# rvp-group/mad-icp

Hardware: NVIDIA H100
Metric: scans/sec (130k-pt scan vs 16-keyframe model) (higher is better)
Workload: dtype f64

## Files before the change

mad_icp_b200/csrc/capi.cu:

```cuda
#include <cooperative_groups.h>
#include <cuda_runtime.h>

#include <algorithm>
#include <cmath>
#include <cstdio>
#include <cstdlib>
#include <cstring>
#include <new>
#include <stdexcept>
#include <string>
#include <vector>

#include "../../include/madicp_b200_debug.h"
#include "ctx.hpp"
#include "device_kernels.cuh"

namespace madicp {

static thread_local std::string g_error;
void set_error(const std::string& msg) { g_error = msg; }

}

using namespace madicp;
// ... 59 lines not shown
  DevPtr<double> ww;
  const size_t total = cap * size_t(c->max_keyframes);
  CK(cudaMalloc(recs.put(), total * sizeof(madtree_rec_t)));
  CK(cudaMalloc(child0.put(), total * sizeof(int)));
  CK(cudaMalloc(rec_of.put(), total * sizeof(int)));
  CK(cudaMalloc(quad.put(), 2 * total * sizeof(QuadRec)));
  CK(cudaMalloc(ww.put(), total * sizeof(double)));
  for (int s = 0; s < c->max_keyframes; ++s)
    if (c->slots[s].n_nodes > 0)
      CK(cudaMemcpyAsync(recs + size_t(s) * cap, c->d_pool_recs + size_t(s) * c->pool_cap,
                         size_t(c->slots[s].n_nodes) * sizeof(madtree_rec_t), cudaMemcpyDeviceToDevice, c->stream));
  CK(cudaStreamSynchronize(c->stream));
  c->d_pool_ww = std::move(ww);
  c->d_pool_recs = std::move(recs);
  c->d_pool_child0 = std::move(child0);
  c->d_pool_rec_of = std::move(rec_of);
  c->d_quad = std::move(quad);
  c->quad_cap = 2 * cap;
  c->pool_cap = cap;
  for (int s = 0; s < c->max_keyframes; ++s)
    if (c->slots[s].n_nodes > 0) {
      int rc = build_slot(c, s, nullptr, nullptr);
      if (rc) return rc;
    }
  return MADICP_OK;
}

static int stage_pose(madicp_ctx* c, const double X[12], const double** X_dev) {
  const int r = int(c->xform_seq % madicp_ctx::kXformRing);
  if (c->xform_seq >= madicp_ctx::kXformRing) CK(cudaEventSynchronize(c->xform_done[r]));
  memcpy(c->h_xform + size_t(r) * 12, X, 12 * sizeof(double));
  CK(cudaMemcpyAsync(c->d_xform + size_t(r) * 12, c->h_xform + size_t(r) * 12, 12 * sizeof(double), cudaMemcpyHostToDevice,
                     c->stream));
  CK(cudaEventRecord(c->xform_done[r], c->stream));
  *X_dev = c->d_xform + size_t(r) * 12;
  c->xform_seq++;
  return MADICP_OK;
}

static int slot_rank(const madicp_ctx* c, int slot) {
  int k = 0;
  for (int s = 0; s < slot; ++s) k += (c->slots[s].n_nodes > 0);
  return k;
}

static int ensure_items(madicp_ctx* c, size_t items) {
  if (items <= c->cap_items) return MADICP_OK;
  CK(cudaStreamSynchronize(c->stream));
  c->cap_items = 0;
  CK(cudaMalloc(c->d_hit.put(), items * sizeof(int)));
  CK(cudaMalloc(c->d_ord.put(), items * sizeof(int)));
  c->cap_items = items;
  return MADICP_OK;
}

struct GnShape {
  int threads, ctas;
  const void* fn;
  size_t smem;
};
template <int THREADS, int CTAS>
static GnShape gn_shape() {
  return GnShape{THREADS, CTAS, reinterpret_cast<const void*>(k_gn_loop<THREADS, CTAS>), gn_dynamic_smem<THREADS>()};
}
static const GnShape* gn_shapes(int* n) {
  static const GnShape table[] = {
      gn_shape<1024, 1>(), gn_shape<896, 1>(), gn_shape<768, 1>(), gn_shape<704, 1>(), gn_shape<640, 1>(),
      gn_shape<512, 1>(),  gn_shape<512, 2>(),
      gn_shape<256, 2>(),  gn_shape<256, 3>(), gn_shape<256, 4>(),
  };
  *n = int(sizeof(table) / sizeof(table[0]));
  return table;
}
static int configure_gn(madicp_ctx* c, int threads, int ctas) {
  int n = 0;
  const GnShape* t = gn_shapes(&n);
  for (int i = 0; i < n; ++i)
    if (t[i].threads == threads && t[i].ctas == ctas) {
      CK(cudaFuncSetAttribute(t[i].fn, cudaFuncAttributeMaxDynamicSharedMemorySize, int(t[i].smem + kGnMapMaxBytes)));
      CK(cudaFuncSetAttribute(t[i].fn, cudaFuncAttributePreferredSharedMemoryCarveout,
                              int((t[i].smem * size_t(ctas) + 2048) * 100 / (228 * 1024)) + 1));
      int per_sm = 0;
      CK(cudaOccupancyMaxActiveBlocksPerMultiprocessor(&per_sm, t[i].fn, threads, t[i].smem));
      if (per_sm < ctas) {
        set_error("persistent kernel shape does not fit on an SM");
        return MADICP_ERR_CUDA;
      }
      c->gn_threads = threads;
      c->gn_grid = ctas * c->sm_count;
      c->gn_kernel = t[i].fn;
      c->gn_smem = t[i].smem;
      return MADICP_OK;
    }
  set_error("unsupported persistent-kernel shape (threads per CTA, CTAs per SM)");
  return MADICP_ERR_INVALID;
}

static int pick_shape(madicp_ctx* c, int64_t items) {
  if (!c->gn_auto) return MADICP_OK;
  const double per_sm = double((items + 31) / 32) / double(c->sm_count);
  int best = 1024;
  double best_cost = 1e300;
  for (int i = 0; i < madicp_ctx::kNumAutoShapes; ++i) {
    const int threads = madicp_ctx::kAutoShapes[i];
    const double passes = ceil(per_sm / double(threads / 32));
    const double cost = passes * c->pass_cost[i];
    if (cost < best_cost) {
      best_cost = cost;
      best = threads;
    }
  }
  if (best == c->gn_threads && c->gn_grid == c->sm_count) return MADICP_OK;
  return configure_gn(c, best, 1);
}

static int grid_for(const madicp_ctx* c, int64_t items) {
  int64_t g = (items + kStepBlock - 1) / kStepBlock;
  const int64_t cap = int64_t(c->sm_count) * 8;
  if (g > cap) g = cap;
  if (g < 1) g = 1;
  return int(g);
}

madicp_ctx::~madicp_ctx() {
  cudaSetDevice(device);
  if (stream) cudaStreamSynchronize(stream);
  for (int r = 0; r < world; ++r)
    if (world > 1 && r != rank && peer_comm[r]) cudaIpcCloseMemHandle(peer_comm[r]);
  madicp_gpu_build_release(this);
  for (madtree_gpu* t : tree_cache) delete t;
  for (CloudBuf* b : cloud_cache) delete b;
}

extern "C" {

const char* madicp_last_error(void) { return g_error.c_str(); }
int madicp_abi_version(void) { return 3; }

int madicp_create(madicp_ctx_t** out, int device, int max_keyframes) {
  if (!out || max_keyframes < 1 || max_keyframes > kMaxSlots) {
    set_error("madicp_create: bad arguments (1 <= max_keyframes <= 64)");
    return MADICP_ERR_INVALID;
  }
  MADICP_TRY
  int n_dev = 0;
  cudaError_t e = cudaGetDeviceCount(&n_dev);
  if (e != cudaSuccess || n_dev <= 0 || device < 0 || device >= n_dev) {
    set_error(std::string("madicp_create: no usable CUDA device (") +
              (e != cudaSuccess ? cudaGetErrorString(e) : "device index out of range") +
              "); this library has no CPU fallback");
    return MADICP_ERR_CUDA;
  }
  CK(cudaSetDevice(device));
  cudaDeviceProp prop;
  CK(cudaGetDeviceProperties(&prop, device));
  if (prop.major != 9 || prop.minor != 0) {
    set_error("madicp_create: device is not sm_90 (H100); kernels are built for sm_90a only");
    return MADICP_ERR_CUDA;
  }
  std::unique_ptr<madicp_ctx> c(new madicp_ctx);
  c->device = device;
  c->max_keyframes = max_keyframes;
  c->sm_count = prop.multiProcessorCount;
  c->slots.resize(max_keyframes);
  {
    int lo_pri = 0, hi_pri = 0;
    CK(cudaDeviceGetStreamPriorityRange(&lo_pri, &hi_pri));
    CK(cudaStreamCreateWithPriority(c->own_stream.put(), cudaStreamNonBlocking, hi_pri));
  }
  c->stream = c->own_stream;
  CK(cudaMalloc(c->d_state.put(), sizeof(GnState)));
  CK(cudaMemset(c->d_state, 0, sizeof(GnState)));
  CK(cudaMalloc(c->d_X.put(), sizeof(double) * 64));
  CK(cudaMalloc(c->d_comm.put(), sizeof(CommBlock)));
// ... 749 lines not shown
  }
  memcpy(c->h_pinned, X, 12 * sizeof(double));
  CK(cudaMemcpyAsync(c->d_X, c->h_pinned, 12 * sizeof(double), cudaMemcpyHostToDevice, c->stream));
  rc = launch_search(c, mv, c->d_X, false);
  if (rc) return rc;
  CK(cudaMemsetAsync(c->d_state, 0, 16, c->stream));
  CK(cudaMemsetAsync(c->d_step_matched, 0, size_t(c->L), c->stream));
  const int64_t items = int64_t(mv.K) * c->L;
  const int grid = grid_for(c, items);
  k_linearize<<<grid, kStepBlock, 0, c->stream>>>(mv, c->d_mov4, c->L, c->d_X, c->P, c->d_hit, c->d_step_matched,
                                                 c->d_partial, c->d_state);
  c->launches++;
  CK(cudaGetLastError());
  CK(cudaMemcpyAsync(c->h_state, c->d_state, offsetof(GnState, X_trace), cudaMemcpyDeviceToHost, c->stream));
  if (matched) CK(cudaMemcpyAsync(c->h_matched, c->d_step_matched, size_t(c->L), cudaMemcpyDeviceToHost, c->stream));
  CK(cudaStreamSynchronize(c->stream));
  memcpy(H, c->h_state->H, sizeof(double) * 36);
  memcpy(b, c->h_state->b, sizeof(double) * 6);
  if (matched) memcpy(matched, c->h_matched, size_t(c->L));
  return MADICP_OK;
}

int madicp_solve_update(madicp_ctx_t* c, const double H[36], const double b[6], double X[12]) {
  if (!c || !H || !b || !X) return MADICP_ERR_INVALID;
  CK(cudaSetDevice(c->device));
  memcpy(c->h_pinned, X, 12 * sizeof(double));
  memcpy(c->h_pinned + 12, H, 36 * sizeof(double));
  memcpy(c->h_pinned + 48, b, 6 * sizeof(double));
  CK(cudaMemcpyAsync(c->d_X, c->h_pinned, 54 * sizeof(double), cudaMemcpyHostToDevice, c->stream));
  k_solve<<<1, 32, 0, c->stream>>>(c->d_X + 12, c->d_X + 48, c->d_X);
  c->launches++;
  CK(cudaGetLastError());
  CK(cudaMemcpyAsync(c->h_pinned, c->d_X, 12 * sizeof(double), cudaMemcpyDeviceToHost, c->stream));
  CK(cudaStreamSynchronize(c->stream));
  memcpy(X, c->h_pinned, 12 * sizeof(double));
  return MADICP_OK;
}

int madicp_debug_inv_det6(madicp_ctx_t* c, const double H[36], double* weight) {
  if (!c || !H || !weight) return MADICP_ERR_INVALID;
  CK(cudaSetDevice(c->device));
  memcpy(c->h_pinned + 12, H, 36 * sizeof(double));
  CK(cudaMemcpyAsync(c->d_X + 12, c->h_pinned + 12, 36 * sizeof(double), cudaMemcpyHostToDevice, c->stream));
  k_inv_det6<<<1, 32, 0, c->stream>>>(c->d_X + 12, c->d_X + 48);
  c->launches++;
  CK(cudaGetLastError());
  CK(cudaMemcpyAsync(c->h_pinned + 48, c->d_X + 48, sizeof(double), cudaMemcpyDeviceToHost, c->stream));
  CK(cudaStreamSynchronize(c->stream));
  *weight = c->h_pinned[48];
  return MADICP_OK;
}

static int register_enqueue(madicp_ctx* c, int iters, const double X0[12], int clear_from) {
  int rc = check_ready(c, "madicp_register");
  if (rc) return rc;
  if (!X0 || iters < 1 || iters > MADICP_MAX_ITERS) {
    set_error("madicp_register: bad arguments (1 <= iters <= 64 per launch)");
    return MADICP_ERR_INVALID;
  }
  CK(cudaSetDevice(c->device));
  rc = prepare_moving(c);
  if (rc) return rc;
  rc = pick_shape(c, int64_t(madicp_num_keyframes(c)) * c->L);
  if (rc) return rc;
  GnArgs A;
  A.model = make_view(c);
  A.P = c->P;
  A.peers.rank = c->rank;
  A.peers.world = c->world;
  A.peers.epoch_base = c->epoch;
  const int mb = int(c->call_seq & 1u);
  for (int r = 0; r < kMaxPeers; ++r) {
    A.peers.box[r] = (r < c->world) ? &c->peer_comm[r]->box : nullptr;
    A.peer_matched[r] = (r < c->world) ? c->peer_comm[r]->matched[mb] : nullptr;
  }
  A.moving = c->d_mov4;
  A.L = c->L;
  A.iters = iters;
  A.clear_from = clear_from;
  A.matched = c->d_comm->matched[mb];
  size_t map_bytes = 0;
  {
    const size_t per_cta = gn_map_bytes(unsigned(madicp_num_keyframes(c)), unsigned(c->L), unsigned(c->gn_grid));
    auto bucket = [](size_t bytes) {
      const size_t kb[] = {8, 16, 32, 64, 100, 132, 164, 196, 228};
      for (size_t b : kb)
        if (bytes + 1024 <= b * 1024) return b;
      return size_t(1 << 20);
    };
    const size_t ctas = size_t(c->gn_grid / c->sm_count);
    if (per_cta && bucket((c->gn_smem + per_cta) * ctas) == bucket(c->gn_smem * ctas)) map_bytes = per_cta;
  }
  A.map_in_smem = map_bytes ? 1 : 0;
  {
    const size_t stride =
        ((size_t(c->max_keyframes) * gn_share_bound(c->cap_moving, unsigned(c->gn_grid))) + 31) & ~size_t(31);
    const size_t need = stride * size_t(c->gn_grid);
    if (need > c->cap_memo) {
      CK(cudaStreamSynchronize(c->stream));
      c->cap_memo = 0;
      const size_t cap = need + need / 4;
      CK(cudaMalloc(c->d_memo_leaf.put(), cap * sizeof(int)));
      CK(cudaMalloc(c->d_memo_margin.put(), cap * sizeof(float)));
      CK(cudaMalloc(c->d_memo_ckpt.put(), cap * sizeof(unsigned)));
      CK(cudaMalloc(c->d_memo_ckpt_up.put(), cap * sizeof(float)));
      c->cap_memo = cap;
    }
    A.memo_leaf = c->d_memo_leaf;
    A.memo_margin = c->d_memo_margin;
    A.memo_ckpt = c->d_memo_ckpt;
    A.memo_ckpt_up = c->d_memo_ckpt_up;
    A.item_stride = int(stride);
    A.memo_mode = c->memo_mode;
    A.walk_buf = mb;
  }
  A.st = c->d_state;
  A.dbg = c->d_dbg;
  A.dbg_cta = c->d_dbg ? c->d_dbg_cta.get() : nullptr;
  c->epoch += uint32_t(iters);
  A.pose_epoch = c->pose_epoch;
  c->pose_epoch += uint32_t(iters);
  memcpy(A.X0, X0, 12 * sizeof(double));
  A.tiles = c->d_tiles;
  A.zero_next = c->d_comm->matched[mb ^ 1];
  A.zero_bytes = int((std::min(kMatchedCap, c->cap_moving) + 15) & ~size_t(15));
  void* args[] = {&A};
  CK(cudaLaunchCooperativeKernel(c->gn_kernel, dim3(c->gn_grid), dim3(c->gn_threads), args, c->gn_smem + map_bytes, c->stream));
  c->launches++;
  c->last_iters = iters;
  c->call_seq++;
  return MADICP_OK;
}

int madicp_register_async(madicp_ctx_t* c, int iters, const double X0[12]) {
  return register_enqueue(c, iters, X0, iters - 1);
}
int madicp_register_partial_async(madicp_ctx_t* c, int iters, const double X0[12]) {
  return register_enqueue(c, iters, X0, 0);
}

int madicp_register_fetch_weight(madicp_ctx_t* c, double X[12], double H[36], double b[6], uint8_t* matched, int* n_matched,
                                 double* weight) {
  if (!c || c->last_iters < 1) {
    set_error("madicp_register_fetch: nothing was enqueued");
    return MADICP_ERR_STATE;
  }
  CK(cudaSetDevice(c->device));
  CK(cudaMemcpyAsync(c->h_state, c->d_state, offsetof(GnState, X_trace), cudaMemcpyDeviceToHost, c->stream));
  if (matched)
    CK(cudaMemcpyAsync(c->h_matched, c->d_comm->matched[(c->call_seq - 1u) & 1u], size_t(c->L), cudaMemcpyDeviceToHost,
                       c->stream));
  CK(cudaStreamSynchronize(c->stream));
  if (c->h_state->error) {
    set_error("madicp_register: a peer GPU never delivered its H/b tile (rank down, or no matching registration enqueued there)");
    CK(cudaMemsetAsync(&c->d_state->error, 0, sizeof(int), c->stream));
    return MADICP_ERR_COMM;
  }
  if (X) memcpy(X, c->h_state->X_out, 12 * sizeof(double));
  if (H) memcpy(H, c->h_state->H, 36 * sizeof(double));
  if (b) memcpy(b, c->h_state->b, 6 * sizeof(double));
  if (matched) memcpy(matched, c->h_matched, size_t(c->L));
  if (n_matched) *n_matched = c->h_state->n_matched;
  if (weight) *weight = c->h_state->weight;
  return MADICP_OK;
}
int madicp_register_fetch(madicp_ctx_t* c, double X[12], double H[36], double b[6], uint8_t* matched, int* n_matched) {
  return madicp_register_fetch_weight(c, X, H, b, matched, n_matched, nullptr);
}

int madicp_register(madicp_ctx_t* c, int iters, double X[12], double H[36], double b[6], uint8_t* matched,
                    int* n_matched) {
  if (!c || !X || iters < 0) {
    set_error("madicp_register: bad arguments");
    return MADICP_ERR_INVALID;
// ... 291 lines not shown
```

mad_icp_b200/csrc/ctx.hpp:

```cpp
#pragma once
#include <cuda_runtime.h>

#include <atomic>
#include <memory>
#include <mutex>
#include <new>
#include <stdexcept>
#include <string>
#include <vector>

#include "cuda_owned.hpp"
#include "kernels.cuh"

namespace madicp {
void set_error(const std::string& msg);

constexpr int kMaxLevels = 4096;
struct Slot {
  int n_nodes = 0, n_leaves = 0, n_levels = 0;
};
constexpr size_t kMatchedCap = size_t(1) << 20;

struct CommBlock {
  Mailbox box;
// ... 24 lines not shown
  std::shared_ptr<madicp::CloudBuf> cloud;
  int64_t cloud_off = 0;
};

struct madicp_ctx {
  ~madicp_ctx();
  int device = 0;
  int max_keyframes = 0;
  madicp::Stream own_stream;
  cudaStream_t stream = nullptr;
  int sm_count = 0;
  std::vector<madicp::Slot> slots;
  size_t pool_cap = 0;
  madicp::DevPtr<madtree_rec_t> d_pool_recs;
  madicp::DevPtr<int> d_pool_child0;
  madicp::DevPtr<int> d_pool_rec_of;
  madicp::DevPtr<int> d_pool_lvl;
  size_t quad_cap = 0;
  madicp::DevPtr<madicp::QuadRec> d_quad;
  madicp::DevPtr<double> d_pool_ww;
  static constexpr int kXformRing = 64;
  madicp::DevPtr<double> d_xform;
  madicp::HostPtr<double> h_xform;
  madicp::HostPtr<int> h_lvl;
  madicp::Event xform_done[kXformRing];
  uint32_t xform_seq = 0;
  static constexpr int kGatherRing = 8;
  madicp::HostPtr<madicp::LeafGather> h_gather;
  madicp::DevPtr<madicp::LeafGather> d_gather;
  size_t cap_gather = 0;
  madicp::Event gather_done[kGatherRing];
  uint32_t gather_seq = 0;
  madicp::DevPtr<double> d_leaves;
  madicp::HostPtr<double> h_leaves;
  size_t cap_leaves = 0;
  std::vector<madtree_gpu*> tree_cache;
  std::vector<madicp::DevPtr<void>> tree_slabs;
  madicp::Event tree_free_ev;
  madicp::Event xstream_ev;
  std::mutex tree_mu;
  bool keep_cloud = false;
  std::vector<madicp::CloudBuf*> cloud_cache;
  std::mutex cloud_mu;
  madicp::HostPtr<int64_t> h_cloud_idx;
  madicp::HostPtr<double> h_cloud_xyz;
  size_t cap_cloud_out = 0;
  void* build_state = nullptr;
  void* plan_state = nullptr;
  madicp::DevPtr<long long> d_dbg_cta;
  madicp::IcpParams P{0.2, 0.31622776601683794, 0.02};
  madicp::DevPtr<double> d_moving;
  madicp::DevPtr<madicp::Moving4> d_mov4;
  bool mov4_stale = true;
  madicp::DevPtr<unsigned char> d_step_matched;
  int L = 0;
  size_t cap_moving = 0;
  uint32_t call_seq = 0;
  madicp::DevPtr<int> d_hit;
  madicp::DevPtr<int> d_ord;
  size_t cap_items = 0;
  madicp::DevPtr<double> d_cloud_q;
  madicp::DevPtr<int> d_cloud_o;
  size_t cap_cloud = 0;
  madicp::DevPtr<double> d_partial;
  madicp::DevPtr<madicp::LLCell> d_tiles;
  size_t cap_partial = 0;
  madicp::DevPtr<int> d_memo_leaf;
  madicp::DevPtr<float> d_memo_margin;
  madicp::DevPtr<unsigned> d_memo_ckpt;
  madicp::DevPtr<float> d_memo_ckpt_up;
  size_t cap_memo = 0;
  int memo_mode = 2;
  madicp::DevPtr<madicp::GnState> d_state;
  madicp::DevPtr<double> d_X;
  madicp::DevPtr<madicp::CommBlock> d_comm;
  madicp::HostPtr<double> h_pinned;
  madicp::HostPtr<madicp::GnState> h_state;
  madicp::HostPtr<unsigned char> h_matched;
  int gn_grid = 0;
  bool gn_auto = true;
  int gn_threads = 1024;
  const void* gn_kernel = nullptr;
  size_t gn_smem = 0;
  static constexpr int kNumAutoShapes = 6;
  static constexpr int kAutoShapes[kNumAutoShapes] = {768, 1024, 896, 704, 640, 512};
  double pass_cost[kNumAutoShapes] = {5570.0, 8260.0, 7480.0, 5650.0, 5325.0, 4650.0};
  bool calibrated = false;
  int last_iters = 0;
  madicp::DevPtr<long long> d_dbg;
  std::atomic<int64_t> launches{0};
  int rank = 0, world = 1;
  madicp::CommBlock* peer_comm[madicp::kMaxPeers] = {};
  uint32_t epoch = 0;
  uint32_t pose_epoch = 1;
};

#define CK(call)                                                                                   \
  do {                                                                                             \
    cudaError_t e_ = (call);                                                                       \
    if (e_ != cudaSuccess) {                                                                       \
      madicp::set_error(std::string(#call) + ": " + cudaGetErrorString(e_));                       \
      return MADICP_ERR_CUDA;                                                                      \
    }                                                                                              \
  } while (0)

#define MADICP_TRY try {
#define MADICP_CATCH(who)                                          \
  }                                                                \
  catch (const std::bad_alloc&) {                                  \
    madicp::set_error(std::string(who) + ": out of host memory");  \
    return MADICP_ERR_NOMEM;                                       \
  }                                                                \
  catch (const std::exception& e_) {                               \
    madicp::set_error(std::string(who) + ": " + e_.what());        \
    return MADICP_ERR_INVALID;                                     \
  }

int madicp_tree_alloc(madicp_ctx* c, size_t cap_nodes, madtree_gpu** out);
int madicp_cloud_alloc(madicp_ctx* c, size_t n, std::shared_ptr<madicp::CloudBuf>* out);
int madicp_check_device_ptr(madicp_ctx* c, const void* p, int align, const char* fn);
int madicp_stream_wait(madicp_ctx* c, void* waiter, void* signaller);
void madicp_gpu_build_release(madicp_ctx* c);
```

mad_icp_b200/csrc/device_kernels.cuh:

```cuda
#pragma once
#include "gn_partition.h"
#include "kernels.cuh"

namespace madicp {


__device__ __forceinline__ int depth_of(const int* __restrict__ lvl, int n_levels, int i) {
  int lo = 0, hi = n_levels;
  while (hi - lo > 1) {
    const int mid = (lo + hi) >> 1;
    if (__ldg(lvl + mid) <= i) lo = mid; else hi = mid;
  }
  return lo;
}

__global__ void __launch_bounds__(kStepBlock)
k_slot_ingest(const madtree_rec_t* src, madtree_rec_t* dst, int n, const double* __restrict__ Xp,
              const int* __restrict__ lvl, int n_levels, int* __restrict__ flag) {
  const int i = blockIdx.x * kStepBlock + threadIdx.x;
  if (i >= n) return;
  Rec r = load_rec_plain(src + i);
  const int npts = src[i].num_points;
  int f = 0;
  if (r.link >= 0 && (depth_of(lvl, n_levels, i) & 1) == 0)
// ... 314 lines not shown
    const double v = s_tot[i];
    const uint32_t lo = uint32_t(__double2loint(v)), hi = uint32_t(__double2hiint(v));
    LLCell* dst = &pv.box[r]->cell[slot][pv.rank][i];
    asm volatile("st.volatile.global.v4.u32 [%0], {%1,%2,%3,%4};" ::"l"(dst), "r"(lo), "r"(epoch), "r"(hi), "r"(epoch)
                 : "memory");
  }
  for (int idx = threadIdx.x; idx < pv.world * kAcc; idx += THREADS) {
    const int r = idx / kAcc, i = idx - r * kAcc;
    const LLCell* src = &pv.box[pv.rank]->cell[slot][r][i];
    uint32_t lo, f0, hi, f1, spins = 0;
    do {
      asm volatile("ld.volatile.global.v4.u32 {%0,%1,%2,%3}, [%4];" : "=r"(lo), "=r"(f0), "=r"(hi), "=r"(f1) : "l"(src)
                   : "memory");
      if (++spins == (1u << 26)) {
        *error = 1;
        break;
      }
    } while (f0 != epoch || f1 != epoch);
    s_peer[r][i] = __hiloint2double(int(hi), int(lo));
  }
  __syncthreads();
  if (threadIdx.x < kAcc) {
    double s = s_peer[0][threadIdx.x];
    for (int r = 1; r < pv.world; ++r) s += s_peer[r][threadIdx.x];
    s_tot[threadIdx.x] = s;
  }
  __syncthreads();
}

struct GnArgs {
  ModelView model;
  IcpParams P;
  PeerView peers;
  const Moving4* moving;
  int L;
  int iters;
  int clear_from;
  unsigned char* matched;
  unsigned char* peer_matched[kMaxPeers];
  LLCell* tiles;
  double X0[12];
  unsigned char* zero_next;
  int zero_bytes;
  GnState* st;
  int map_in_smem;
  uint32_t pose_epoch;
  int* memo_leaf;
  float* memo_margin;
  unsigned* memo_ckpt;
  float* memo_ckpt_up;
  int item_stride;
  int walk_buf;
  int memo_mode;
  long long* dbg;
  long long* dbg_cta;
};
#ifndef MADICP_CKPT_TAU_SCALE
#define MADICP_CKPT_TAU_SCALE 1.0
#endif
__device__ __forceinline__ float ckpt_tau(int it, double moved, double ball) {
  return __double2float_ru(MADICP_CKPT_TAU_SCALE * (it == 0 ? ball : moved));
}

__device__ __forceinline__ long long global_ns() {
  long long t;
  asm volatile("mov.u64 %0, %%globaltimer;" : "=l"(t));
  return t;
}

template <int THREADS, int CTAS>
__global__ void __launch_bounds__(THREADS, CTAS)
k_gn_loop(const __grid_constant__ GnArgs A) {
  constexpr int WARPS = THREADS / 32;
  extern __shared__ __align__(16) double s_dyn[];
  double* s_stage_all = s_dyn;
  double(*s_red)[64] = reinterpret_cast<double(*)[64]>(s_dyn);
  double(*s_peer)[kAcc] = reinterpret_cast<double(*)[kAcc]>(s_dyn + WARPS * 64);
  static_assert(WARPS * 64 + kMaxPeers * kAcc <= WARPS * kStageTile, "scratch must fit in the staging tiles");
  __shared__ double s_tot[kAcc];
  __shared__ double s_b[6];
  __shared__ double s_X[12], s_Xp[12];
  __shared__ int s_qn, s_rn;
  __shared__ int s_count[WARPS];
  GnState* st = A.st;
  const unsigned L = unsigned(A.L);
  const unsigned total = unsigned(A.model.K) * L;
  const bool multi = A.peers.world > 1;
  const unsigned lane = threadIdx.x & 31;
  const unsigned warp = threadIdx.x >> 5;
  double* stage = s_stage_all + warp * kStageTile;
  constexpr unsigned kPieces = kGnPieces;
  unsigned p_lo[kPieces], p_n[kPieces];
  unsigned n_b = 0;
#pragma unroll
  for (unsigned p = 0; p < kPieces; ++p) {
    gn_stretch(L, gridDim.x, blockIdx.x, p, p_lo[p], p_n[p]);
    n_b += p_n[p];
  }
  const unsigned t_total = unsigned(A.model.K) * n_b;
  (void) total;
  auto item_of = [&](unsigned t0, unsigned& k, unsigned& q) {
    k = t0 / n_b;
    q = t0 - k * n_b + lane;
    while (q >= n_b) {
      q -= n_b;
      ++k;
    }
    const unsigned j = q;
    q = p_lo[kPieces - 1] + (j - (n_b - p_n[kPieces - 1]));
    unsigned acc = 0;
#pragma unroll
    for (unsigned p = 0; p + 1 < kPieces; ++p) {
      if (j >= acc && j < acc + p_n[p]) q = p_lo[p] + (j - acc);
      acc += p_n[p];
    }
  };
  unsigned* s_map = A.map_in_smem ? reinterpret_cast<unsigned*>(s_dyn + WARPS * kStageTile) : nullptr;
  if (s_map) {
    for (unsigned t0 = warp * 32; t0 < t_total; t0 += THREADS) {
      unsigned k, q;
      item_of(t0, k, q);
      s_map[t0 + lane] = (k << 26) | q;
    }
    __syncwarp();
  }

  for (int i = (blockIdx.x * THREADS + threadIdx.x) * 16; i < A.zero_bytes; i += gridDim.x * THREADS * 16)
    *reinterpret_cast<uint4*>(A.zero_next + i) = make_uint4(0, 0, 0, 0);
  if (blockIdx.x == 0 && threadIdx.x < MADICP_MAX_ITERS) {
    st->walked[A.walk_buf ^ 1][threadIdx.x] = 0;
    st->walk_recs[A.walk_buf ^ 1][threadIdx.x] = 0;
  }
  int* const memo_leaf = A.memo_leaf + size_t(blockIdx.x) * A.item_stride;
  float* const memo_margin = A.memo_margin + size_t(blockIdx.x) * A.item_stride;
  unsigned* const memo_ckpt = A.memo_ckpt + size_t(blockIdx.x) * A.item_stride;
  float* const memo_ckpt_up = A.memo_ckpt_up + size_t(blockIdx.x) * A.item_stride;
  auto item_at = [&](unsigned t0, unsigned& k, unsigned& q) {
    if (s_map) {
      const unsigned pk = s_map[t0 + lane];
      k = pk >> 26;
      q = pk & 0x3ffffffu;
    } else {
      item_of(t0, k, q);
    }
  };

  for (int it = 0; it < A.iters; ++it) {
    if (threadIdx.x < 12) {
      double x;
      if (it == 0) {
        x = A.X0[threadIdx.x];
      } else {
        const uint32_t ep = A.pose_epoch + uint32_t(it);
        uint32_t lo, hi, f0, f1;
        do {
          ll_load(&st->X_ll[threadIdx.x], lo, f0, hi, f1);
        } while (f0 != ep || f1 != ep);
        x = __hiloint2double(int(hi), int(lo));
      }
      s_Xp[threadIdx.x] = s_X[threadIdx.x];
      s_X[threadIdx.x] = x;
      if (it == 0 && blockIdx.x == 0) st->X_trace[threadIdx.x] = x;
    }
    if (threadIdx.x == 32) s_qn = 0;
    if (threadIdx.x == 33) s_rn = 0;
    __syncthreads();
    const bool last_round = (it == A.iters - 1);
    double c0 = 0.0, c1 = 0.0;
    long long t_begin = 0;
    if (A.dbg && threadIdx.x == 0) t_begin = clock64();
    const size_t dbg_plane = size_t(MADICP_MAX_ITERS) * gridDim.x, dbg_at = size_t(it) * gridDim.x + blockIdx.x;
    if (A.dbg_cta && threadIdx.x == 0) A.dbg_cta[dbg_plane + dbg_at] = global_ns();

    int n_walked = 0, n_recs = 0;
    for (unsigned t0 = warp * 32; t0 < t_total; t0 += THREADS) {
      unsigned k, q;
      item_at(t0, k, q);
      double v[kStage];
#pragma unroll
      for (int i = 0; i < kStage; ++i) v[i] = 0.0;
      const unsigned t = t0 + lane;
      if (t < t_total) {
        const Moving4 m = load_moving(A.moving + q);
        double mx, my, mz;
        iso_apply(s_X, m.px, m.py, m.pz, mx, my, mz);
        int leaf = -1;
        Rec f;
        double ww = 0.0;
        unsigned start = 0;
        float prefix = __int_as_float(0x7f800000);
        double moved = 0.0;
        if (it > 0 && A.memo_mode) {
          const float have = memo_margin[t];
          const int last = memo_leaf[t];
          unsigned ck = 0;
          float ck_up = 0.0f;
          if (A.memo_mode == 2) {
            ck = memo_ckpt[t];
            ck_up = memo_ckpt_up[t];
          }
          f = load_rec(A.model.recs + last);
          ww = __ldg(A.model.ww + last);
          double bx, by, bz;
          iso_apply(s_Xp, m.px, m.py, m.pz, bx, by, bz);
          const double dx = mx - bx, dy = my - by, dz = mz - bz;
          moved = 1.0001 * sqrt(dx * dx + dy * dy + dz * dz) + 1e-9 + 1e-12 * (fabs(mx) + fabs(my) + fabs(mz));
          const double left = double(have) - moved;
          if (left > 0.0) {
            memo_margin[t] = __double2float_rd(left);
            leaf = last;
          } else if (ck != 0) {
            const double ck_left = __dsub_rd(__dadd_rd(double(have), double(ck_up)), moved);
            if (ck_left > 0.0) {
              start = ck;
              prefix = __double2float_rd(ck_left);
            }
          }
        }
        if (leaf < 0) {
          double ww_walk;
          const float tau = ckpt_tau(it, moved, m.ball);
          float margin = prefix, ck_margin = 0.0f;
          unsigned ckpt = start;
          leaf = A.memo_mode ? descend_t<true>(A.model, int(k), mx, my, mz, ww_walk, margin, ckpt, ck_margin, tau, n_recs)
                             : descend_t<false>(A.model, int(k), mx, my, mz, ww_walk, margin, ckpt, ck_margin, tau, n_recs);
          if (A.memo_mode) {
            memo_leaf[t] = leaf;
            memo_margin[t] = margin;
          }
          if (A.memo_mode == 2) {
            memo_ckpt[t] = ckpt;
            memo_ckpt_up[t] = __fsub_rd(ck_margin, margin);
          }
          ++n_walked;
          ww = __ldg(A.model.ww + leaf);
          f = load_rec(A.model.recs + leaf);
        }
        if (linearize_one(s_X, A.P.rho_ker_sqrt, m, mx, my, mz, f, ww, v) && it >= A.clear_from) {
          if (multi) {
            for (int r = 0; r < A.peers.world; ++r) A.peer_matched[r][q] = 1;
          } else {
            A.matched[q] = 1;
          }
        }
      }
      warp_accumulate(stage, v, c0, c1);
    }
    n_walked = __reduce_add_sync(0xffffffffu, n_walked);
    n_recs = __reduce_add_sync(0xffffffffu, n_recs);
    if (lane == 0 && n_walked) {
      atomicAdd(&s_qn, n_walked);
      atomicAdd(&s_rn, n_recs);
    }
    if (A.dbg && threadIdx.x == 0 && blockIdx.x == 0) A.dbg[it * 8 + 0] = clock64() - t_begin;
    if (A.dbg_cta) {
      __syncthreads();
      if (threadIdx.x == 0) {
        A.dbg_cta[dbg_at] = clock64() - t_begin;
        A.dbg_cta[2 * dbg_plane + dbg_at] = global_ns();
      }
      if (threadIdx.x == 0 && blockIdx.x == 0) A.dbg[it * 8 + 5] = s_qn;
    }
    __syncthreads();
    if (threadIdx.x == 0 && s_qn) {
      atomicAdd(&st->walked[A.walk_buf][it], s_qn);
      atomicAdd(&st->walk_recs[A.walk_buf][it], (unsigned long long) s_rn);
    }
    const uint32_t ep_round = A.pose_epoch + uint32_t(it);
    block_reduce_publish<WARPS>(c0, c1, s_red, A.tiles + size_t(blockIdx.x) * kAcc, ep_round,
                                 it >= A.clear_from, multi);
    if (A.dbg_cta && threadIdx.x == 0) A.dbg_cta[3 * dbg_plane + dbg_at] = global_ns();
    if (blockIdx.x == 0) {
      long long t0 = 0, t1 = 0, t2 = 0;
      if (A.dbg && threadIdx.x == 0) t0 = clock64();
      fold_tiles<THREADS>(A.tiles, gridDim.x, ep_round, s_red, s_tot,
                          (A.dbg_cta && gridDim.x >= 16) ? A.dbg_cta + 4 * dbg_plane + size_t(it) * gridDim.x : nullptr);
      if (A.dbg && threadIdx.x == 0) {
        t1 = clock64();
        A.dbg[it * 8 + 1] = t1 - t_begin;
        A.dbg[it * 8 + 2] = t1 - t0;
        A.dbg[it * 8 + 6] = global_ns();
      }
      if (multi) {
        if (last_round) __threadfence_system();
        peer_allreduce<THREADS>(A.peers, A.peers.epoch_base + uint32_t(it) + 1u, s_tot, s_peer, &st->error);
        if (last_round) __threadfence_system();
      }
      if (last_round) {
        __threadfence();
        int c = 0;
        {
          const uint4* m16 = reinterpret_cast<const uint4*>(A.matched);
          for (int q = threadIdx.x; q < (A.L + 15) / 16; q += THREADS) {
            const uint4 w = __ldcv(m16 + q);
            c += __popc(w.x) + __popc(w.y) + __popc(w.z) + __popc(w.w);
          }
        }
        for (int off = 16; off > 0; off >>= 1) c += __shfl_down_sync(0xffffffffu, c, off);
        if (lane == 0) s_count[warp] = c;
      }
      if (threadIdx.x < 6) s_b[threadIdx.x] = s_tot[threadIdx.x * 8 + 6];
      __syncthreads();
      if (last_round && threadIdx.x >= 32) {
        if (threadIdx.x == 32) unpack_Hb(s_tot, st->H, st->b);
        if (threadIdx.x == 64) st->weight = inv_det6_dev(s_tot, 8);
        if (threadIdx.x == 96) {
          int c = 0;
          for (int w2 = 0; w2 < WARPS; ++w2) c += s_count[w2];
          st->n_matched = c;
        }
      }
      if (threadIdx.x == 0) {
        if (A.dbg) t2 = clock64();
        double Xn[12];
        gn_update_pose(s_tot, 8, s_b, s_X, Xn);
        if (!last_round) {
          const uint32_t ep = ep_round + 1u;
#pragma unroll
          for (int i = 0; i < 12; ++i) ll_store(&st->X_ll[i], Xn[i], ep);
        }
#pragma unroll
// ... 22 lines not shown
```

mad_icp_b200/csrc/kernels.cuh:

```cuda
#pragma once
#include <cuda_runtime.h>
#include <stdint.h>

#include "../../include/madicp_b200.h"
#include "arith.h"
#include "solve6.h"

namespace madicp {

constexpr int kMaxSlots = 64;
constexpr int kStepBlock = 256;
constexpr int kAcc = 48;
constexpr int kStage = 13;
constexpr int kStageItems = 16;
constexpr int kStagePitch = 20;
constexpr int kStageTile = kStage * kStagePitch;
constexpr int kMaxPeers = 16;
constexpr int kMailboxSlots = 2;

struct __align__(16) FastRec {
  float dx, dy, dz, c;
};
static_assert(sizeof(FastRec) == 16, "FastRec must be one 128-bit load");

constexpr float kBoundC = 1.0e-6f;

struct __align__(32) QuadRec {
  FastRec p0, p1, p2;
  int bfs0;
  int child0;
  int pad[2];
};
static_assert(sizeof(QuadRec) == 64, "QuadRec must be four 128-bit loads");

struct ModelView {
  const madtree_rec_t* recs;
  const QuadRec* quad;
  const double* ww;
  int broot[kMaxSlots];
  int qroot[kMaxSlots];
  int K;
};
constexpr unsigned kLeafMarker = 0x7fc0beefu;

struct IcpParams {
  double min_ball, rho_ker_sqrt, b_ratio;
};

struct __align__(32) Moving4 {
  double px, py, pz, ball;
};

struct LeafGather {
  const madtree_rec_t* recs;
  const int* leaf_of;
  int out, n_leaves, has_pose, pad;
  double X[12];
};

struct CloudOut {
  const double* xyz;
  const int32_t* idx;
  long long n;
  int has_pose, pad;
  double X[12];
};

struct __align__(16) LLCell {
  uint32_t lo, flag_lo, hi, flag_hi;
};

__device__ __forceinline__ void ll_store(LLCell* p, double v, uint32_t epoch) {
  asm volatile("st.volatile.global.v4.u32 [%0], {%1,%2,%3,%4};" ::"l"(p), "r"(uint32_t(__double2loint(v))), "r"(epoch),
               "r"(uint32_t(__double2hiint(v))), "r"(epoch) : "memory");
}
__device__ __forceinline__ void ll_load(const LLCell* p, uint32_t& lo, uint32_t& f0, uint32_t& hi, uint32_t& f1) {
  asm volatile("ld.volatile.global.v4.u32 {%0,%1,%2,%3}, [%4];" : "=r"(lo), "=r"(f0), "=r"(hi), "=r"(f1) : "l"(p) : "memory");
}

struct GnState {
  int ticket;
  int clear_from;
  int n_matched;
  int error;
  double X_in[12];
  double X_out[12];
  double H[36];
  double b[6];
  double weight;
  double X_trace[(MADICP_MAX_ITERS + 1) * 12];
  int walked[2][MADICP_MAX_ITERS];
  unsigned long long walk_recs[2][MADICP_MAX_ITERS];
  LLCell X_ll[12];
};

struct Mailbox {
// ... 105 lines not shown
  const QueryF q = make_query(qx, qy, qz);
  const unsigned qroot = unsigned(M.qroot[k]);
  const QuadRec* qbase = M.quad;
  unsigned g = qroot + ckpt;
  if (MEMO) ckpt_margin = margin;
  while (true) {
    if (MEMO && margin >= tau) {
      ckpt = g - qroot;
      ckpt_margin = margin;
    }
    ++n_rec;
    FastRec p0, p1, p2;
    int bfs0, child0, pad1, pad2;
    const char* rp = reinterpret_cast<const char*>(qbase + g);
    ld_nc_f32x4(rp, p0.dx, p0.dy, p0.dz, p0.c);
    ld_nc_f32x4(rp + 16, p1.dx, p1.dy, p1.dz, p1.c);
    ld_nc_f32x4(rp + 32, p2.dx, p2.dy, p2.dz, p2.c);
    ld_nc_s32x4(rp + 48, bfs0, child0, pad1, pad2);
    if (is_leaf(p0)) {
      ww = leaf_weight(p0);
      return leaf_index(p0);
    }
    const SideF f0 = side_filtered2(q, p0);
    bool s0 = f0.right;
    if (MEMO) {
      float mg = f0.margin;
      if (!f0.decided) {
        const float r = side_exact_m(M.recs + bfs0, qx, qy, qz);
        s0 = exact_right(r);
        mg = fabsf(r);
      }
      margin = fminf(margin, mg);
    } else if (!f0.decided) {
      s0 = side_exact(M.recs + bfs0, qx, qy, qz);
    }
    const FastRec c = s0 ? p2 : p1;
    if (is_leaf(c)) {
      ww = leaf_weight(c);
      return leaf_index(c);
    }
    const SideF f1 = side_filtered2(q, c);
    bool s1 = f1.right;
    if (MEMO) {
      float mg = f1.margin;
      if (!f1.decided) {
        const float r = side_exact_m(M.recs + (M.broot[k] + load_rec_link(M.recs + bfs0) + (s0 ? 1 : 0)), qx, qy, qz);
        s1 = exact_right(r);
        mg = fabsf(r);
      }
      margin = fminf(margin, mg);
    } else if (!f1.decided) {
      s1 = side_exact(M.recs + (M.broot[k] + load_rec_link(M.recs + bfs0) + (s0 ? 1 : 0)), qx, qy, qz);
    }
    g = qroot + unsigned(child0) + (s0 ? 2u : 0u) + (s1 ? 1u : 0u);
  }
}

__device__ __forceinline__ int descend(const ModelView& M, int k, double qx, double qy, double qz, double& ww) {
  float unused = 0.0f, unused_ck = 0.0f;
  unsigned root = 0;
  int unused_n = 0;
  return descend_t<false>(M, k, qx, qy, qz, ww, unused, root, unused_ck, 0.0f, unused_n);
}

__device__ __forceinline__ bool linearize_one(const double* __restrict__ X, double rho, const Moving4& m, double mlx,
                                              double mly, double mlz, const Rec& f, double ww, double* v) {
  const double ex = mlx - f.mx, ey = mly - f.my, ez = mlz - f.mz;
  const double d2 = dot3(ex, ey, ez, ex, ey, ez);
  const double b2 = m.ball * fabs(m.ball);
  if (d2 > b2 * (1.0 + 1e-14)) return false;
  if (!(d2 < b2 * (1.0 - 1e-14)) && sqrt(d2) > m.ball) return false;
  const double e = fma(ez, f.dz, fma(ey, f.dy, ex * f.dx));
  double J[6];
  J[0] = fma(f.dz, X[8], fma(f.dy, X[4], f.dx * X[0]));
  J[1] = fma(f.dz, X[9], fma(f.dy, X[5], f.dx * X[1]));
  J[2] = fma(f.dz, X[10], fma(f.dy, X[6], f.dx * X[2]));
  J[3] = fma(J[2], m.py, -(J[1] * m.pz));
  J[4] = fma(J[0], m.pz, -(J[2] * m.px));
  J[5] = fma(J[1], m.px, -(J[0] * m.py));
  double scale = ww;
  const double chi = fabs(e);
  if (chi > rho) scale = (rho / chi) * ww;
#pragma unroll
  for (int i = 0; i < 6; ++i) {
    v[i] = scale * J[i];
    v[6 + i] = J[i];
  }
  v[12] = e;
  return true;
}

__device__ __forceinline__ void warp_accumulate(double* stage, const double* v, double& c0, double& c1) {
  const int lane = threadIdx.x & 31;
  const int g = lane >> 2, t = lane & 3;
#pragma unroll
  for (int h = 0; h < 2; ++h) {
    if ((lane >> 4) == h) {
#pragma unroll
      for (int i = 0; i < kStage; ++i) stage[i * kStagePitch + (lane & 15)] = v[i];
    }
    __syncwarp();
#pragma unroll
    for (int s = 0; s < 4; ++s) {
      const double* it = stage + (4 * s + t);
      const double a = (g < 6) ? it[g * kStagePitch] : 0.0;
      const double b = (g < 7) ? it[(6 + (g < 7 ? g : 6)) * kStagePitch] : 0.0;
      asm volatile("mma.sync.aligned.m8n8k4.row.col.f64.f64.f64.f64 {%0,%1}, {%2}, {%3}, {%0,%1};"
                   : "+d"(c0), "+d"(c1)
                   : "d"(a), "d"(b));
    }
    __syncwarp();
  }
}

template <int WARPS>
__device__ __forceinline__ void block_reduce_store(double c0, double c1, double (*s_red)[64], double* out) {
  const int lane = threadIdx.x & 31, warp = threadIdx.x >> 5;
  const int g = lane >> 2, t = lane & 3;
  s_red[warp][g * 8 + 2 * t] = c0;
  s_red[warp][g * 8 + 2 * t + 1] = c1;
  __syncthreads();
  if (threadIdx.x < kAcc) {
    double s = s_red[0][threadIdx.x];
#pragma unroll
    for (int w2 = 1; w2 < WARPS; ++w2) s += s_red[w2][threadIdx.x];
    out[threadIdx.x] = s;
  }
}

template <int WARPS>
__device__ __forceinline__ void block_reduce_publish(double c0, double c1, double (*s_red)[64], LLCell* out, uint32_t epoch,
                                                     bool fence, bool system_scope) {
  const int lane = threadIdx.x & 31, warp = threadIdx.x >> 5;
  const int g = lane >> 2, t = lane & 3;
  s_red[warp][g * 8 + 2 * t] = c0;
  s_red[warp][g * 8 + 2 * t + 1] = c1;
  __syncthreads();
  if (threadIdx.x < kAcc) {
    double s = s_red[0][threadIdx.x];
#pragma unroll
    for (int w2 = 1; w2 < WARPS; ++w2) s += s_red[w2][threadIdx.x];
    if (fence) {
      if (system_scope) __threadfence_system(); else __threadfence();
    }
    ll_store(out + threadIdx.x, s, epoch);
  }
}

template <int THREADS>
__device__ __forceinline__ void fold_tiles(const LLCell* tiles, int nblk, uint32_t epoch, double (*s_red)[64], double* s_tot,
                                           long long* trace = nullptr) {
  int n_sweeps = 0;
  if (trace && threadIdx.x == 0) trace[0] = clock64();
  constexpr int STRANDS = THREADS / kAcc > 16 ? 16 : THREADS / kAcc;
  constexpr int kPer = 10;
  const int j = (threadIdx.x < STRANDS * kAcc) ? int(threadIdx.x % kAcc) : 64, g = threadIdx.x / kAcc;
  __syncthreads();
  if (j < kAcc) {
    double s = 0.0;
    for (int blk0 = g; blk0 < nblk; blk0 += kPer * STRANDS) {
      double v[kPer];
      unsigned missing = 0;
#pragma unroll
      for (int i = 0; i < kPer; ++i) {
        v[i] = 0.0;
        if (blk0 + i * STRANDS < nblk) missing |= 1u << i;
      }
      while (missing) {
        uint32_t lo[kPer], hi[kPer], f0[kPer], f1[kPer];
#pragma unroll
        for (int i = 0; i < kPer; ++i) {
          f0[i] = f1[i] = ~epoch;
          lo[i] = hi[i] = 0;
          if (missing & (1u << i)) ll_load(tiles + size_t(blk0 + i * STRANDS) * kAcc + j, lo[i], f0[i], hi[i], f1[i]);
        }
        if (trace && threadIdx.x == 0) {
          if (n_sweeps < 12) trace[1 + n_sweeps] = clock64();
          ++n_sweeps;
        }
#pragma unroll
        for (int i = 0; i < kPer; ++i)
          if ((missing & (1u << i)) && f0[i] == epoch && f1[i] == epoch) {
            v[i] = __hiloint2double(int(hi[i]), int(lo[i]));
            missing &= ~(1u << i);
          }
      }
#pragma unroll
      for (int i = 0; i < kPer; ++i) s += v[i];
    }
// ... 75 lines not shown
```

Measured before the change: 4982.

## Shrink staged linearization rows and move per-item state out of registers

Each warp now stages 8 values per match (J, residual, robust scale) instead of 13, and forms the weighted row in the MMA operand load instead of storing scale*J separately. This cuts shared-memory staging per warp. Piece bounds move from per-thread arrays into shared memory, and memo pointers become one base offset. The leaf record and moving point are now loaded once after the memo/descend branch rather than held across it, which should lower register pressure. The smem-bucket check now counts static shared memory, and the auto-shape table drops 1024 threads and gets new pass costs.

Result: faster. 5352, median of 6 (+7.4%).

```diff
diff --git a/mad_icp_b200/csrc/capi.cu b/mad_icp_b200/csrc/capi.cu
--- a/mad_icp_b200/csrc/capi.cu
+++ b/mad_icp_b200/csrc/capi.cu
@@ -165,6 +165,8 @@
                               int((t[i].smem * size_t(ctas) + 2048) * 100 / (228 * 1024)) + 1));
       int per_sm = 0;
       CK(cudaOccupancyMaxActiveBlocksPerMultiprocessor(&per_sm, t[i].fn, threads, t[i].smem));
+      cudaFuncAttributes fa;
+      CK(cudaFuncGetAttributes(&fa, t[i].fn));
       if (per_sm < ctas) {
         set_error("persistent kernel shape does not fit on an SM");
         return MADICP_ERR_CUDA;
@@ -173,6 +175,7 @@
       c->gn_grid = ctas * c->sm_count;
       c->gn_kernel = t[i].fn;
       c->gn_smem = t[i].smem;
+      c->gn_static_smem = fa.sharedSizeBytes;
       return MADICP_OK;
     }
   set_error("unsupported persistent-kernel shape (threads per CTA, CTAs per SM)");
@@ -1088,14 +1091,15 @@
   size_t map_bytes = 0;
   {
     const size_t per_cta = gn_map_bytes(unsigned(madicp_num_keyframes(c)), unsigned(c->L), unsigned(c->gn_grid));
-    auto bucket = [](size_t bytes) {
+    const size_t ctas = size_t(c->gn_grid / c->sm_count);
+    auto bucket = [&](size_t dynamic) {
+      const size_t bytes = ctas * (dynamic + c->gn_static_smem + 1024);
       const size_t kb[] = {8, 16, 32, 64, 100, 132, 164, 196, 228};
       for (size_t b : kb)
-        if (bytes + 1024 <= b * 1024) return b;
+        if (bytes <= b * 1024) return b;
       return size_t(1 << 20);
     };
-    const size_t ctas = size_t(c->gn_grid / c->sm_count);
-    if (per_cta && bucket((c->gn_smem + per_cta) * ctas) == bucket(c->gn_smem * ctas)) map_bytes = per_cta;
+    if (per_cta && bucket(c->gn_smem + per_cta) == bucket(c->gn_smem)) map_bytes = per_cta;
   }
   A.map_in_smem = map_bytes ? 1 : 0;
   {
diff --git a/mad_icp_b200/csrc/ctx.hpp b/mad_icp_b200/csrc/ctx.hpp
--- a/mad_icp_b200/csrc/ctx.hpp
+++ b/mad_icp_b200/csrc/ctx.hpp
@@ -130,9 +130,10 @@
   int gn_threads = 1024;
   const void* gn_kernel = nullptr;
   size_t gn_smem = 0;
-  static constexpr int kNumAutoShapes = 6;
-  static constexpr int kAutoShapes[kNumAutoShapes] = {768, 1024, 896, 704, 640, 512};
-  double pass_cost[kNumAutoShapes] = {5570.0, 8260.0, 7480.0, 5650.0, 5325.0, 4650.0};
+  size_t gn_static_smem = 0;
+  static constexpr int kNumAutoShapes = 5;
+  static constexpr int kAutoShapes[kNumAutoShapes] = {768, 896, 704, 640, 512};
+  double pass_cost[kNumAutoShapes] = {4935.0, 6195.0, 5060.0, 4925.0, 4165.0};
   bool calibrated = false;
   int last_iters = 0;
   madicp::DevPtr<long long> d_dbg;
diff --git a/mad_icp_b200/csrc/device_kernels.cuh b/mad_icp_b200/csrc/device_kernels.cuh
--- a/mad_icp_b200/csrc/device_kernels.cuh
+++ b/mad_icp_b200/csrc/device_kernels.cuh
@@ -420,6 +420,7 @@
   __shared__ double s_X[12], s_Xp[12];
   __shared__ int s_qn, s_rn;
   __shared__ int s_count[WARPS];
+  __shared__ unsigned s_plo[kGnPieces], s_pn[kGnPieces];
   GnState* st = A.st;
   const unsigned L = unsigned(A.L);
   const unsigned total = unsigned(A.model.K) * L;
@@ -428,13 +429,18 @@
   const unsigned warp = threadIdx.x >> 5;
   double* stage = s_stage_all + warp * kStageTile;
   constexpr unsigned kPieces = kGnPieces;
-  unsigned p_lo[kPieces], p_n[kPieces];
   unsigned n_b = 0;
 #pragma unroll
   for (unsigned p = 0; p < kPieces; ++p) {
-    gn_stretch(L, gridDim.x, blockIdx.x, p, p_lo[p], p_n[p]);
-    n_b += p_n[p];
-  }
+    unsigned lo, n;
+    gn_stretch(L, gridDim.x, blockIdx.x, p, lo, n);
+    if (threadIdx.x == 0) {
+      s_plo[p] = lo;
+      s_pn[p] = n;
+    }
+    n_b += n;
+  }
+  __syncthreads();
   const unsigned t_total = unsigned(A.model.K) * n_b;
   (void) total;
   auto item_of = [&](unsigned t0, unsigned& k, unsigned& q) {
@@ -445,12 +451,13 @@
       ++k;
     }
     const unsigned j = q;
-    q = p_lo[kPieces - 1] + (j - (n_b - p_n[kPieces - 1]));
+    q = s_plo[kPieces - 1] + (j - (n_b - s_pn[kPieces - 1]));
     unsigned acc = 0;
 #pragma unroll
     for (unsigned p = 0; p + 1 < kPieces; ++p) {
-      if (j >= acc && j < acc + p_n[p]) q = p_lo[p] + (j - acc);
-      acc += p_n[p];
+      const unsigned n = s_pn[p];
+      if (j >= acc && j < acc + n) q = s_plo[p] + (j - acc);
+      acc += n;
     }
   };
   unsigned* s_map = A.map_in_smem ? reinterpret_cast<unsigned*>(s_dyn + WARPS * kStageTile) : nullptr;
@@ -469,10 +476,7 @@
     st->walked[A.walk_buf ^ 1][threadIdx.x] = 0;
     st->walk_recs[A.walk_buf ^ 1][threadIdx.x] = 0;
   }
-  int* const memo_leaf = A.memo_leaf + size_t(blockIdx.x) * A.item_stride;
-  float* const memo_margin = A.memo_margin + size_t(blockIdx.x) * A.item_stride;
-  unsigned* const memo_ckpt = A.memo_ckpt + size_t(blockIdx.x) * A.item_stride;
-  float* const memo_ckpt_up = A.memo_ckpt_up + size_t(blockIdx.x) * A.item_stride;
+  const unsigned memo0 = blockIdx.x * unsigned(A.item_stride);
   auto item_at = [&](unsigned t0, unsigned& k, unsigned& q) {
     if (s_map) {
       const unsigned pk = s_map[t0 + lane];
@@ -523,29 +527,25 @@
         double mx, my, mz;
         iso_apply(s_X, m.px, m.py, m.pz, mx, my, mz);
         int leaf = -1;
-        Rec f;
-        double ww = 0.0;
         unsigned start = 0;
         float prefix = __int_as_float(0x7f800000);
         double moved = 0.0;
         if (it > 0 && A.memo_mode) {
-          const float have = memo_margin[t];
-          const int last = memo_leaf[t];
+          const float have = A.memo_margin[memo0 + t];
+          const int last = A.memo_leaf[memo0 + t];
           unsigned ck = 0;
           float ck_up = 0.0f;
           if (A.memo_mode == 2) {
-            ck = memo_ckpt[t];
-            ck_up = memo_ckpt_up[t];
+            ck = A.memo_ckpt[memo0 + t];
+            ck_up = A.memo_ckpt_up[memo0 + t];
           }
-          f = load_rec(A.model.recs + last);
-          ww = __ldg(A.model.ww + last);
           double bx, by, bz;
           iso_apply(s_Xp, m.px, m.py, m.pz, bx, by, bz);
           const double dx = mx - bx, dy = my - by, dz = mz - bz;
           moved = 1.0001 * sqrt(dx * dx + dy * dy + dz * dz) + 1e-9 + 1e-12 * (fabs(mx) + fabs(my) + fabs(mz));
           const double left = double(have) - moved;
           if (left > 0.0) {
-            memo_margin[t] = __double2float_rd(left);
+            A.memo_margin[memo0 + t] = __double2float_rd(left);
             leaf = last;
           } else if (ck != 0) {
             const double ck_left = __dsub_rd(__dadd_rd(double(have), double(ck_up)), moved);
@@ -563,18 +563,19 @@
           leaf = A.memo_mode ? descend_t<true>(A.model, int(k), mx, my, mz, ww_walk, margin, ckpt, ck_margin, tau, n_recs)
                              : descend_t<false>(A.model, int(k), mx, my, mz, ww_walk, margin, ckpt, ck_margin, tau, n_recs);
           if (A.memo_mode) {
-            memo_leaf[t] = leaf;
-            memo_margin[t] = margin;
+            A.memo_leaf[memo0 + t] = leaf;
+            A.memo_margin[memo0 + t] = margin;
           }
           if (A.memo_mode == 2) {
-            memo_ckpt[t] = ckpt;
-            memo_ckpt_up[t] = __fsub_rd(ck_margin, margin);
+            A.memo_ckpt[memo0 + t] = ckpt;
+            A.memo_ckpt_up[memo0 + t] = __fsub_rd(ck_margin, margin);
           }
           ++n_walked;
-          ww = __ldg(A.model.ww + leaf);
-          f = load_rec(A.model.recs + leaf);
-        }
-        if (linearize_one(s_X, A.P.rho_ker_sqrt, m, mx, my, mz, f, ww, v) && it >= A.clear_from) {
+        }
+        const double ww = __ldg(A.model.ww + leaf);
+        const Rec f = load_rec(A.model.recs + leaf);
+        const Moving4 m2 = load_moving(A.moving + q);
+        if (linearize_one(s_X, A.P.rho_ker_sqrt, m2, mx, my, mz, f, ww, v) && it >= A.clear_from) {
           if (multi) {
             for (int r = 0; r < A.peers.world; ++r) A.peer_matched[r][q] = 1;
           } else {
diff --git a/mad_icp_b200/csrc/kernels.cuh b/mad_icp_b200/csrc/kernels.cuh
--- a/mad_icp_b200/csrc/kernels.cuh
+++ b/mad_icp_b200/csrc/kernels.cuh
@@ -11,7 +11,7 @@
 constexpr int kMaxSlots = 64;
 constexpr int kStepBlock = 256;
 constexpr int kAcc = 48;
-constexpr int kStage = 13;
+constexpr int kStage = 8;
 constexpr int kStageItems = 16;
 constexpr int kStagePitch = 20;
 constexpr int kStageTile = kStage * kStagePitch;
@@ -283,11 +283,9 @@
   const double chi = fabs(e);
   if (chi > rho) scale = (rho / chi) * ww;
 #pragma unroll
-  for (int i = 0; i < 6; ++i) {
-    v[i] = scale * J[i];
-    v[6 + i] = J[i];
-  }
-  v[12] = e;
+  for (int i = 0; i < 6; ++i) v[i] = J[i];
+  v[6] = e;
+  v[7] = scale;
   return true;
 }
 
@@ -304,8 +302,8 @@
 #pragma unroll
     for (int s = 0; s < 4; ++s) {
       const double* it = stage + (4 * s + t);
-      const double a = (g < 6) ? it[g * kStagePitch] : 0.0;
-      const double b = (g < 7) ? it[(6 + (g < 7 ? g : 6)) * kStagePitch] : 0.0;
+      const double b = (g < 7) ? it[g * kStagePitch] : 0.0;
+      const double a = (g < 6) ? it[7 * kStagePitch] * b : 0.0;
       asm volatile("mma.sync.aligned.m8n8k4.row.col.f64.f64.f64.f64 {%0,%1}, {%2}, {%3}, {%0,%1};"
                    : "+d"(c0), "+d"(c1)
                    : "d"(a), "d"(b));
```
